# sandialabs/PyNucleus

Hardware: AMD Instinct MI355X
Metric: element-pairs/sec assembled (2D P1 fractional s=0.5, dense) + % fp64 roofline (higher is better)
Workload: dtype f64; 1 GPU; 2D unit disc (uniform_disc refined 7x, 98304 cells), P1, 48769 DoFs, fractional s=0.5, horizon=inf, dense getDense incl. zeroExterior; 4831887360 element pairs/step; noRef=7, num_dofs=48769, num_cells=98304, parallelism=block rows of the upper triangle dealt over 1 GPU(s), row-owned one-sided slabs

## Files before the change

### include/pnl_hip.h

```cpp
#ifndef PNL_HIP_H
#define PNL_HIP_H
#include <stdint.h>

#ifdef __cplusplus
extern "C" {
#endif

typedef struct pnl_context pnl_context;

enum pnl_status {
    PNL_OK = 0,
    PNL_ERR_INVALID = -1,
    PNL_ERR_UNSUPPORTED = -2,
    PNL_ERR_HIP = -3,
    PNL_ERR_STATE = -4,
    PNL_ERR_ORDER = -5
};

enum pnl_kernel_type { PNL_FRACTIONAL = 0, PNL_INDICATOR = 1, PNL_PERIDYNAMIC = 2, PNL_GAUSSIAN = 3, PNL_EXPONENTIAL = 4,
                       PNL_GAUSSIAN_BOUNDARY = 5, PNL_EXPONENTIAL_BOUNDARY = 6 };

typedef struct {
    int32_t ktype;
    int32_t interaction;
// ... 117 lines not shown
int pnl_h2_get(pnl_context *ctx, int which, double *dst_host);
int pnl_h2_set(pnl_context *ctx, int which, const double *src_host);
int pnl_h2_matvec_block(pnl_context *ctx, int nvec, const double *X_dev, int64_t ldx, double *Y_dev, int64_t ldy);
int pnl_h2_upward_block(pnl_context *ctx, int nvec, const double *X_dev, int64_t ldx, double *cupB_dev);
int pnl_h2_interact_block(pnl_context *ctx, const double *cupB_dev, double *cdownB_dev);
int pnl_h2_downward_block(pnl_context *ctx, int nvec, double *cdownB_dev, double *Y_dev, int64_t ldy);

int pnl_spmv(pnl_context *ctx, const double *data_dev, const double *diag_dev, const double *x_dev, double *y_dev);

typedef struct pnl_order_function {
    int32_t type, normalized;
    double p[6];
    int32_t scal_n, pad;
    double scal_mid, scal_half;
    double scal_cheb[32];
} pnl_order_function;

int pnl_set_order_function(pnl_context *ctx, const pnl_order_function *f, const double *cell_smax, const double *facet_smax,
                           double c0, double bc0, double sing_fac, double bsing_fac);
int pnl_set_order_vertex_values(pnl_context *ctx, int nv, const double *values_host);
int pnl_upload_pointwise_rules(pnl_context *ctx, int which, int panel, int nkeys, int M, int rows, const double *nodes,
                               const double *w, const double *phi0, const double *phi1);
int pnl_assemble_dense_pointwise(pnl_context *ctx, double *A, int64_t ldA, int zero_exterior, int cell_begin, int cell_end,
                                 int npairs, const int32_t *pairs, int nbpairs, const int32_t *bpairs);
int pnl_assemble_pairs_masked_pointwise(pnl_context *ctx, int np, const int32_t *pairs, const uint64_t *masks, const int32_t *rule,
                                        double *data);
int pnl_assemble_boundary_masked_pointwise(pnl_context *ctx, int ni, const int32_t *cells, const int32_t *facets, const uint32_t *masks,
                                           const int32_t *rule, const double *sv, double fac, double *data, double *diag);

int pnl_get_counters(pnl_context *ctx, int64_t *out, int n);
int pnl_get_phase_ms(pnl_context *ctx, float *out, int n);
int pnl_get_settled_tiles(pnl_context *ctx, int32_t *tiles, int64_t ntiles);
int pnl_get_settled_lists(pnl_context *ctx, uint16_t *codes, uint16_t *lists, int64_t ntiles);
int pnl_uniform_lane_layout(int nc, const int32_t *cells, const int32_t *dofs, int mode, int nthreads, int32_t *sizes, uint8_t *lane_cell,
                            int16_t *lds_col, int8_t *vorder, int16_t *cell_col, double *mult, double *seconds);
enum pnl_kernel_slot { PNL_K_TILE_GENERAL = 0, PNL_K_TILE_UNIFORM2, PNL_K_TILE_UNIFORM3, PNL_K_TILE_UNIFORM4, PNL_K_FOLD_MIRROR,
                       PNL_K_WORKLIST, PNL_K_TILE_SETTLED, PNL_NUM_KERNEL_SLOTS };
int pnl_get_kernel_ms(pnl_context *ctx, float *out, int n);

typedef struct pnl_tree pnl_tree;
typedef struct pnl_nfplan pnl_nfplan;
int pnl_tree_build(int N, int dim, const double *boxes, const int64_t *d2c_ptr, const int32_t *d2c_idx, int nc, double eta,
                   int min_size, int max_levels, int do_admissibility, pnl_tree **out);
int pnl_tree_build_blocks(int N, int dim, const double *boxes, const int64_t *d2c_ptr, const int32_t *d2c_idx, int nc, double eta,
                          int min_size, int max_levels, int do_admissibility, const int32_t *dof_block, int mixed_block,
                          pnl_tree **out);
int pnl_tree_build_refined(int N, int dim, const double *boxes, const int64_t *d2c_ptr, const int32_t *d2c_idx, int nc, double eta,
                           int min_size, int max_levels, int do_admissibility, const int32_t *dof_block, int mixed_block, int ref_type,
                           pnl_tree **out);
int pnl_tree_build_horizon(int N, int dim, const double *boxes, const int64_t *d2c_ptr, const int32_t *d2c_idx, int nc, double eta,
                           int min_size, int max_levels, int do_admissibility, const int32_t *dof_block, int mixed_block, int ref_type,
                           double horizon, pnl_tree **out);
int pnl_tree_build_device(int N, int dim, const double *boxes, const int64_t *d2c_ptr, const int32_t *d2c_idx, int nc, double eta,
                          int min_size, int max_levels, int do_admissibility, int ref_type, pnl_tree **out);
void pnl_tree_destroy(pnl_tree *T);
int pnl_tree_sizes(const pnl_tree *T, int64_t *out3);
int pnl_tree_get(const pnl_tree *T, int32_t *range, int32_t *parent, int32_t *children, int32_t *level, double *box, int32_t *perm,
                 int32_t *near, int32_t *far);
int pnl_tree_node_cells(const pnl_tree *T, int n, const int32_t *node_ids, int64_t *off, int32_t *cells);
int pnl_h2_transfer_matrices(int nnodes, int dim, int m, const double *box, const int32_t *parent, double *out);
int pnl_nfplan_build(int dim, int nv, const double *vertices, int nc, const int32_t *cells, int dpe, int N, const int32_t *dofs,
                     int nnodes, const int64_t *node_off, const int32_t *node_dofs, const int64_t *node_cell_off,
                     const int32_t *node_cells, int npairs, const int32_t *pair_nodes, int tile, int max_chunk_dofs,
                     pnl_nfplan **out);
void pnl_nfplan_destroy(pnl_nfplan *P);
int pnl_nfplan_sizes(const pnl_nfplan *P, int64_t *out9);
// ... 123 lines not shown
```

### pynucleus_amd/_lib.py

```python
import ctypes as C
import os
import numpy as np

_HERE = os.path.dirname(os.path.abspath(__file__))
LIB_PATH = os.environ.get('PNL_LIB', os.path.join(_HERE, 'libpnl_hip.so'))

PNL_OK = 0
PNL_ERR_INVALID = -1
PNL_ERR_UNSUPPORTED = -2
PNL_ERR_HIP = -3
PNL_ERR_STATE = -4
PNL_ERR_ORDER = -5
PNL_INTERIOR = 0
PNL_BOUNDARY = 1
PNL_FLAG_NO_MIRROR = 1
PNL_FLAG_SYMMETRIC_FLUSH = 2
PNL_NUM_COUNTERS = 140

EXPORTS = ['pnl_create', 'pnl_destroy', 'pnl_error_string', 'pnl_version', 'pnl_set_stream', 'pnl_synchronize',
           'pnl_upload_mesh', 'pnl_upload_dofmap', 'pnl_set_kernel', 'pnl_set_order_formula', 'pnl_upload_distant_rules',
           'pnl_upload_singular_rule', 'pnl_upload_boundary', 'pnl_assemble_dense', 'pnl_dense_overwrites', 'pnl_block_row_costs', 'pnl_tile_cells',
           'pnl_assemble_dense_tiles', 'pnl_get_counters', 'pnl_get_phase_ms', 'pnl_get_kernel_ms', 'pnl_get_settled_tiles', 'pnl_tree_build', 'pnl_tree_build_blocks', 'pnl_tree_build_refined', 'pnl_tree_build_horizon', 'pnl_tree_build_device', 'pnl_tree_destroy', 'pnl_tree_sizes', 'pnl_tree_get', 'pnl_tree_node_cells', 'pnl_h2_transfer_matrices', 'pnl_nfplan_build', 'pnl_nfplan_destroy', 'pnl_nfplan_sizes', 'pnl_nfplan_get', 'pnl_horizon_pattern', 'pnl_near_pattern', 'pnl_pattern_set_max_nnz', 'pnl_set_option', 'pnl_set_cell_order', 'pnl_set_interaction_transform', 'pnl_set_order_vertex_values', 'pnl_h2_get', 'pnl_h2_set', 'pnl_pattern_nnz', 'pnl_pattern_get', 'pnl_pattern_destroy', 'pnl_set_row_slab', 'pnl_diag_blocks_size', 'pnl_get_diag_blocks', 'pnl_slab_matvec', 'pnl_slab_diagonal', 'pnl_gemv', 'pnl_cg_jacobi',
           'pnl_inv_diagonal', 'pnl_set_classes', 'pnl_select_class', 'pnl_upload_sparsity', 'pnl_upload_sparsity_device', 'pnl_assemble_pairs_masked', 'pnl_assemble_boundary_masked', 'pnl_assemble_clusters_tiled', 'pnl_h2_setup', 'pnl_h2_matvec', 'pnl_h2_upward', 'pnl_h2_interact', 'pnl_h2_downward', 'pnl_h2_sizes', 'pnl_spmv',
           'pnl_assemble_pairs_in_horizon', 'pnl_assemble_pairs_in_horizon_range', 'pnl_set_nonsymmetric', 'pnl_set_order_function', 'pnl_upload_pointwise_rules', 'pnl_assemble_dense_pointwise',
           'pnl_assemble_pairs_masked_pointwise', 'pnl_assemble_boundary_masked_pointwise', 'pnl_get_settled_lists',
           'pnl_gemv_axpby', 'pnl_csr_matvec', 'pnl_mg_create', 'pnl_mg_destroy', 'pnl_mg_cycle', 'pnl_mg_solve', 'pnl_mg_cg', 'pnl_theta_step', 'pnl_selftest',
           'pnl_potrf', 'pnl_potrs', 'pnl_getrf', 'pnl_getrs',
           'pnl_csr_cg_jacobi', 'pnl_fe_space_create', 'pnl_fe_space_destroy', 'pnl_assemble_nonlinearity', 'pnl_imex_create',
           'pnl_imex_destroy', 'pnl_imex_sweep', 'pnl_lincomb', 'pnl_gemv_multi', 'pnl_gemv_block', 'pnl_spmv_block', 'pnl_uniform_lane_layout',
           'pnl_h2_matvec_block', 'pnl_h2_upward_block', 'pnl_h2_interact_block', 'pnl_h2_downward_block',
           'pnl_cg_jacobi_block', 'pnl_cgb_init', 'pnl_cgb_update', 'pnl_cgb_refresh', 'pnl_cgb_direction']

PNL_FUN_BRUSSELATOR, PNL_FUN_CUBIC = 0, 1
PNL_IMEX_CG_MG, PNL_IMEX_CHOL = 0, 1
PNL_IMEX_MAX_STAGES, PNL_IMEX_MAX_COMP = 4, 2
PNL_INTERP_MAX_OPS = 21
PNL_CGB_MAXVEC, PNL_CGB_STATE = 16, 8


def source_sha16():
    import glob
    import hashlib
    root = os.path.dirname(_HERE)
    files = sorted(glob.glob(os.path.join(_HERE, 'csrc', '*.h'))+glob.glob(os.path.join(_HERE, 'csrc', '*.hip'))
                   +[os.path.join(root, 'include', 'pnl_hip.h'), os.path.join(_HERE, 'csrc', 'Makefile')])
    h = hashlib.sha256()
    for fn in files:
        with open(fn, 'rb') as f:
            h.update(os.path.basename(fn).encode()+b'\0'+f.read())
    return h.hexdigest()[:16]


class pnl_kernel(C.Structure):
    _fields_ = [('ktype', C.c_int32), ('interaction', C.c_int32), ('exponent', C.c_double), ('scale', C.c_double),
                ('horizon2', C.c_double)]


class pnl_order_formula(C.Structure):
# ... 54 lines not shown
        return _LIB
    if not os.path.exists(LIB_PATH):
        raise PnlError('{} is missing: the HIP extension has not been built (run __graft_entry__.build()); '
                       'there is no CPU fallback for the assembly path'.format(LIB_PATH))
    import torch
    L = C.CDLL(LIB_PATH)
    vp, i32, i64, dbl = C.c_void_p, C.c_int, C.c_int64, C.c_double
    L.pnl_create.argtypes = [i32, C.POINTER(vp)]
    L.pnl_destroy.argtypes = [vp]
    L.pnl_destroy.restype = None
    L.pnl_error_string.argtypes = [vp]
    L.pnl_error_string.restype = C.c_char_p
    L.pnl_version.restype = C.c_char_p
    L.pnl_set_stream.argtypes = [vp, vp]
    L.pnl_synchronize.argtypes = [vp]
    L.pnl_upload_mesh.argtypes = [vp, i32, i32, vp, i32, vp, vp, vp, dbl]
    L.pnl_upload_dofmap.argtypes = [vp, i32, i32, i32, i32, vp, vp]
    L.pnl_set_kernel.argtypes = [vp, i32, C.POINTER(pnl_kernel)]
    L.pnl_selftest.argtypes = [i32, i32, i32, i32, vp, i32, vp, vp]
    L.pnl_set_order_formula.argtypes = [vp, i32, C.POINTER(pnl_order_formula)]
    L.pnl_upload_distant_rules.argtypes = [vp, i32, vp, vp, vp, vp, vp, vp, vp]
    L.pnl_upload_singular_rule.argtypes = [vp, i32, i32, i32, i32, vp, vp, vp, dbl]
    L.pnl_upload_boundary.argtypes = [vp, i32, vp]
    L.pnl_assemble_dense.argtypes = [vp, vp, i64, i32, i32, i32, i32]
    L.pnl_dense_overwrites.argtypes = [vp, i32, i32, i32]
    L.pnl_block_row_costs.argtypes = [vp, vp, i32]
    L.pnl_tile_cells.argtypes = [vp]
    L.pnl_assemble_dense_tiles.argtypes = [vp, vp, i64, i32, i32, vp, i32, i32, i32]
    L.pnl_get_counters.argtypes = [vp, vp, i32]
    L.pnl_get_phase_ms.argtypes = [vp, vp, i32]
    L.pnl_get_kernel_ms.argtypes = [vp, vp, i32]
    L.pnl_get_settled_tiles.argtypes = [vp, vp, C.c_int64]
    L.pnl_get_settled_lists.argtypes = [vp, vp, vp, C.c_int64]
    L.pnl_uniform_lane_layout.argtypes = [i32, vp, vp, i32, i32, vp, vp, vp, vp, vp, vp, vp]
    L.pnl_set_row_slab.argtypes = [vp, i32, vp, i32, vp]
    L.pnl_tree_build.argtypes = [i32, i32, vp, vp, vp, i32, dbl, i32, i32, i32, C.POINTER(vp)]
    L.pnl_tree_build_blocks.argtypes = [i32, i32, vp, vp, vp, i32, dbl, i32, i32, i32, vp, i32, C.POINTER(vp)]
    L.pnl_tree_build_refined.argtypes = [i32, i32, vp, vp, vp, i32, dbl, i32, i32, i32, vp, i32, i32, C.POINTER(vp)]
    L.pnl_tree_build_horizon.argtypes = [i32, i32, vp, vp, vp, i32, dbl, i32, i32, i32, vp, i32, i32, dbl, C.POINTER(vp)]
    L.pnl_tree_build_device.argtypes = [i32, i32, vp, vp, vp, i32, dbl, i32, i32, i32, i32, C.POINTER(vp)]
    L.pnl_tree_destroy.argtypes = [vp]
    L.pnl_tree_destroy.restype = None
    L.pnl_tree_sizes.argtypes = [vp, vp]
    L.pnl_tree_get.argtypes = [vp, vp, vp, vp, vp, vp, vp, vp, vp]
    L.pnl_tree_node_cells.argtypes = [vp, i32, vp, vp, vp]
    L.pnl_h2_transfer_matrices.argtypes = [i32, i32, i32, vp, vp, vp]
    L.pnl_nfplan_build.argtypes = [i32, i32, vp, i32, vp, i32, i32, vp, i32, vp, vp, vp, vp, i32, vp, i32, i32, C.POINTER(vp)]
    L.pnl_nfplan_destroy.argtypes = [vp]
    L.pnl_nfplan_destroy.restype = None
    L.pnl_nfplan_sizes.argtypes = [vp, vp]
    L.pnl_nfplan_get.argtypes = [vp, i32, vp]
    L.pnl_horizon_pattern.argtypes = [i32, i32, vp, i32, vp, i32, i32, vp, dbl, i32, C.POINTER(vp)]
    L.pnl_near_pattern.argtypes = [vp, i32, vp, i32, C.POINTER(vp)]
    L.pnl_pattern_nnz.argtypes = [vp]
    L.pnl_pattern_set_max_nnz.argtypes = [i64]
    L.pnl_set_option.argtypes = [C.c_char_p, C.c_char_p]
    L.pnl_set_cell_order.argtypes = [vp, i32, vp]
    L.pnl_set_interaction_transform.argtypes = [vp, i32, vp]
    L.pnl_set_order_vertex_values.argtypes = [vp, i32, vp]
    L.pnl_h2_get.argtypes = [vp, i32, vp]
    L.pnl_h2_set.argtypes = [vp, i32, vp]
    L.pnl_pattern_get.argtypes = [vp, vp, vp]
    L.pnl_pattern_destroy.argtypes = [vp]
    L.pnl_diag_blocks_size.argtypes = [vp]
    L.pnl_get_diag_blocks.argtypes = [vp, vp]
    L.pnl_slab_matvec.argtypes = [vp, vp, i64, vp, vp, vp]
# ... 409 lines not shown
        self.check(self.L.pnl_get_diag_blocks(self.h, C.c_void_p(dst_ptr)))

    def slab_matvec(self, slab_ptr, ld, dblocks_ptr, x_ptr, y_ptr):
        self.check(self.L.pnl_slab_matvec(self.h, C.c_void_p(slab_ptr), int(ld), C.c_void_p(dblocks_ptr), C.c_void_p(x_ptr), C.c_void_p(y_ptr)))

    def slab_diagonal(self, slab_ptr, ld, dblocks_ptr, diag_ptr):
        self.check(self.L.pnl_slab_diagonal(self.h, C.c_void_p(slab_ptr), int(ld), C.c_void_p(dblocks_ptr), C.c_void_p(diag_ptr)))

    def kernel_ms(self):
        out = np.zeros(7, dtype=np.float32)
        self.check(self.L.pnl_get_kernel_ms(self.h, out.ctypes.data, 7))
        return dict(tile_general=float(out[0]), tile_uniform2=float(out[1]), tile_uniform3=float(out[2]), tile_uniform4=float(out[3]),
                    fold_mirror=float(out[4]), worklist=float(out[5]), tile_settled=float(out[6]))

    def settled_tiles(self):
        n = self.L.pnl_get_settled_tiles(self.h, None, 0)
        self.check(min(n, 0))
        tiles = np.zeros((n, 2), dtype=np.int32)
        if n:
            self.check(min(self.L.pnl_get_settled_tiles(self.h, tiles.ctypes.data, n), 0))
        return tiles

    def settled_lists(self):
        n = self.settled_tiles().shape[0]
        codes = np.zeros((n, 512), dtype=np.uint16)
        have = self.L.pnl_get_settled_lists(self.h, codes.ctypes.data if n else None, None, n)
        self.check(min(have, 0))
        if not have:
            return codes, None
        lists = np.zeros((n, 4104), dtype=np.uint16)
        self.check(min(self.L.pnl_get_settled_lists(self.h, None, lists.ctypes.data, n), 0))
        return codes, lists

    def gemv(self, A_ptr, ldA, n, x_ptr, y_ptr, symmetric_half=False):
        self.check(self.L.pnl_gemv(self.h, C.c_void_p(A_ptr), int(ldA), int(n), C.c_void_p(x_ptr), C.c_void_p(y_ptr),
                                   int(symmetric_half)))

    def cg_jacobi(self, A_ptr, ldA, n, b_ptr, x_ptr, tol, maxiter):
        it, res = C.c_int(0), C.c_double(0.)
        self.check(self.L.pnl_cg_jacobi(self.h, C.c_void_p(A_ptr), int(ldA), int(n), C.c_void_p(b_ptr), C.c_void_p(x_ptr),
                                        float(tol), int(maxiter), C.byref(it), C.byref(res)))
        return it.value, res.value

    def gemv_axpby(self, A_ptr, ldA, nrows, ncols, x_ptr, alpha, beta, b_ptr, y_ptr):
        self.check(self.L.pnl_gemv_axpby(self.h, C.c_void_p(A_ptr), int(ldA), int(nrows), int(ncols), C.c_void_p(x_ptr), float(alpha),
                                         float(beta), C.c_void_p(b_ptr) if b_ptr else None, C.c_void_p(y_ptr)))

    @staticmethod
    def _block_list(A_ptrs, coeffs):
        c = np.ascontiguousarray(coeffs, dtype=np.float64)
        assert c.ndim == 1 and c.shape[0] == len(A_ptrs)
        return (C.c_void_p*max(len(A_ptrs), 1))(*[int(p) if p else None for p in A_ptrs]), c

    def lincomb(self, A_ptrs, ldA, nrows, ncols, coeffs, B_ptr, ldB):
        arr, c = self._block_list(A_ptrs, coeffs)
        self.check(self.L.pnl_lincomb(self.h, len(A_ptrs), arr, int(ldA), int(nrows), int(ncols), c.ctypes.data, C.c_void_p(B_ptr) if B_ptr else None,
                                      int(ldB)))

    def gemv_multi(self, A_ptrs, ldA, nrows, ncols, coeffs, x_ptr, alpha, beta, b_ptr, y_ptr):
        arr, c = self._block_list(A_ptrs, coeffs)
        self.check(self.L.pnl_gemv_multi(self.h, len(A_ptrs), arr, int(ldA), int(nrows), int(ncols), c.ctypes.data, C.c_void_p(x_ptr), float(alpha),
                                         float(beta), C.c_void_p(b_ptr) if b_ptr else None, C.c_void_p(y_ptr)))

    def gemv_block(self, A_ptr, ldA, nrows, ncols, nvec, X_ptr, ldx, alpha, beta, B_ptr, ldb, Y_ptr, ldy):
        self.check(self.L.pnl_gemv_block(self.h, C.c_void_p(A_ptr) if A_ptr else None, int(ldA), int(nrows), int(ncols), int(nvec),
                                         C.c_void_p(X_ptr) if X_ptr else None, int(ldx), float(alpha), float(beta),
# ... 139 lines not shown
```

### pynucleus_amd/csrc/pnl_context.h

```cpp
#pragma once
#include <hip/hip_runtime.h>
#include <algorithm>
#include <cmath>
#include <cstdarg>
#include <cstdio>
#include <cstring>
#include <string>
#include <vector>
#include "pnl_hip.h"
#include "pnl_device.h"

constexpr int TILE_P1 = 64;
constexpr int TILE_P2 = 32;

struct DevBuf {
    void *p = nullptr;
    size_t bytes = 0;
    ~DevBuf() { release(); }
    void release() { if (p) { (void)hipFree(p); p = nullptr; bytes = 0; } }
};

enum PhaseEvent {
    EV_START = 0,
    EV_WORKLIST_DONE = 1,
// ... 45 lines not shown
    double H0 = 0.;
    std::vector<double> vertices, vol, h;
    std::vector<int32_t> cells, dofs, perm_table, bcells;
    struct ClassData {
        pnl_kernel kern[2];
        pnl_order_formula form[2];
        bool have_kernel[2] = {false, false}, have_form[2] = {false, false};
        bool have_sing[2][3] = {{false, false, false}, {false, false, false}};
        DevBuf b_sn[3], b_sw[3], b_sp[3], b_bn[2], b_bw[2], b_bp[2], b_spairs[3], b_bpairs[2], b_spairs1[3];
        int sM[3] = {0, 0, 0}, sRows[3] = {0, 0, 0}, bM[2] = {0, 0};
        double sFac = 0., bFac = 0.;
        int n_spairs[3] = {0, 0, 0}, n_bpairs[2] = {0, 0};
        int n_spairs1[3] = {0, 0, 0};
        ClassData() { std::memset(kern, 0, sizeof(kern)); std::memset(form, 0, sizeof(form)); }
    };
    std::vector<ClassData*> cls;
    int cur = 0;
    ClassData &C() { return *cls[cur]; }
    int nlab = 0;
    bool nonsym = false;
    int orient = 0;
    std::vector<int32_t> cell_labels, facet_labels, cls_of;
    bool have_mesh = false, have_dofs = false, have_rules = false, have_boundary = false;
    bool dirty = true;
    DevProblem P;
    DevBuf b_cellv, b_ccen, b_cvol, b_ch, b_clog, b_cvid, b_cdof, b_cslot, b_blk_ndof, b_blk_dofs, b_perm, b_off, b_bary, b_w, b_phi,
        b_foff, b_fbary, b_fw, b_bvid, b_bv, b_bgeo, b_counters, b_D, b_tiles,
        b_vec[6], b_clabel, b_blabel, b_clsof, b_scal, b_wl, b_wlcount, b_tilectr, b_ttn, b_ttoff, b_tttab, b_ttwphi, b_wlsorted, b_wlaux,
        b_vertices, b_sp_indptr, b_sp_indices, b_mp_pairs, b_mp_masks, b_mp_wl, b_mp_sorted, b_mp_aux, b_bi_cells, b_bi_facets,
        b_bi_masks, b_cp[28], b_cpD, b_wlds, b_wlpair, b_h2[27];
    DevBuf b_kcls, b_fcls, b_uni, b_tilecls, b_ttwphif;
    DevBuf b_scolbase, b_srowoff, b_cpoff, b_cpslot, b_cprow, b_foldtab, b_bkcls, b_bfcls, b_bdefer, b_multitiles, b_slotA, b_candtiles, b_candq;
    int slot_S = 0, n_multitiles = 0;
    DevBuf b_codes, b_lists;
    int n_settled = 0, settled_want = -1, lists_want = -1;
    std::vector<int2> settled_tiles;
    long long code_builds = 0;
    DevBuf b_unictr;
    static constexpr int UNI_CTRS = 64;
    long long slot_total = 0;
    DevBuf b_rowmap, b_rowdof, b_colmap, b_coldof;
    DevBuf b_cholinfo;
    DevBuf b_luwork, b_lutmp;
    DevBuf b_blk_part, b_blk_xt;
    DevBuf b_cgb_part, b_cgb_work;
    std::vector<int32_t> slab_rowdofs, slab_coldofs;
    int slab_rows = 0, slab_cols = 0;
    std::vector<DevKernel> kcls_host;
    std::vector<DevKernel> bkcls_host;
    std::vector<DevFormula> bfcls_host;
    std::vector<DevFormula> fcls_host;
    int uni_off[5] = {-1, -1, -1, -1, -1}, uni_np[5] = {0, 0, 0, 0, 0};
    bool uni_struct[5] = {false, false, false, false, false};
    H2Dev h2;
    bool have_h2 = false;
    bool have_tile_order = false;
    struct TileOrderJob *tile_job = nullptr;
    DevBuf b_cellv_t, b_cdof_t, b_cslot_t, b_Dt;
    UniLaneTables uni_lanes[3];
    int uni_lanes_up = -1;
    double uni_lanes_seconds = 0.;
    DevBuf b_ul_cell, b_ul_col, b_ul_ccol, b_ul_cellv, b_ul_cvol, b_ul_cslot, b_ul_real;
    std::vector<double> ul_cellv_t;
    std::vector<short> ul_cslot_t;
    PwDev pw;
    bool have_pw = false, have_pw_rules[2][3] = {{false, false, false}, {false, false, false}};
// ... 236 lines not shown
```

### pynucleus_amd/csrc/pnl_device.h

```cpp
#pragma once
#include <hip/hip_runtime.h>
#include <stdint.h>

#define PNL_NTHREADS 256
#define PNL_MAXQ 120
#define PNL_NCOUNTERS 136
#define PNL_DC_UNI_TILES_UNCHECKED 134
#define PNL_DC_UNI_TILES_CHECKED 135
#define PNL_WL_SLOTS 256
#define PNL_WL_BINS 128
#define PNL_POW_TAB_DOUBLES 384
#define PNL_TT_MAXPTS 96
#define PNL_GEN_MAXPTS 16

struct DevKernel {
    int ktype;
    int fast;
    double exponent, scale, horizon2;
    int interaction, qm;
    double pb[6];
    const double *ptab;
};

struct DevFormula {
// ... 32 lines not shown
    const double *tt_wphi;
    const double *tt_wphif;
    int tt_npts, pad1;
    int sM[3], sRows[3];
    const double *sNodes[3], *sW[3], *sPsi[3];
    double sFac;
    int bM[2];
    const double *bNodes[2], *bW[2], *bPhi[2];
    double bFac;
    const int *bvid;
    const double *bv;
    const double *bgeo;
    const int *clabel, *blabel, *cls_of;
    int nlab, cur_class;
    int orient, pad2;
    double idfac;
    unsigned long long *counters;
    const int *rowmap, *colmap;
    int onesided, pad3;
    const double *uni = nullptr;
    int uni_off[5] = {0, 0, 0, 0, 0};
    int mix_struct = 0;
};

constexpr int PNL_DIAG_MULT = 21;
#define PNL_LIST_HEAD 8
#define PNL_LIST_STRIDE (PNL_LIST_HEAD+4096)
__host__ __device__ constexpr int tile_sweep_row(int tid, int k, int tile, int nt) { return k*(nt/tile)+tid/tile; }
__host__ __device__ constexpr int tile_diag_cell(int r, int j, int tile) { return (r+PNL_DIAG_MULT*j)%tile; }

__device__ __forceinline__ long long pnl_row(const DevProblem &P, int I) { return P.rowmap ? (long long)P.rowmap[I] : (long long)I; }
__device__ __forceinline__ int pnl_col(const DevProblem &P, int J) { return P.colmap ? P.colmap[J] : J; }

#define PNL_FOLD_TAB 63
struct FoldEntry { long long off; int ar, cy; };

struct H2Dev {
    int dim, m, M, nnodes, nleaves, nfar;
    const double *box;
    const int *parent;
    const int *leaf_node;
    const int *leaf_dof_off, *leaf_dofs;
    const int *leaf_cell_off, *leaf_cells;
    const long long *leaf_val_off;
    const int *far;
    double *V, *K;
    const double *T;
    double *cup, *cdown;
};

__device__ __forceinline__ double cheb_node(double a, double b, int m, int j) {
    return (b-a)*0.5*(cos((2.0*(m-j)-1.0)/(2.0*m)*3.14159265358979323846)+1.0)+a;
}

__device__ __forceinline__ double lagrange1d(double a, double b, int m, int l, double x) {
    const double xl = cheb_node(a, b, m, l);
    double v = 1.;
    for (int k = 0; k < m; k++)
        if (k != l) {
            const double xk = cheb_node(a, b, m, k);
            v *= (x-xk)/(xl-xk);
        }
    return v;
}

struct PwDev {
    int type, normalized;
// ... 38 lines not shown
```

### pynucleus_amd/csrc/pnl_setup.hip

```cpp
#include <hip/hip_runtime.h>
#include <algorithm>
#include <chrono>
#include <cmath>
#include <cstdio>
#include <cstring>
#include <deque>
#include <map>
#include <mutex>
#include <string>
#include <thread>
#include <vector>
#include "pnl_hip.h"
#include "pnl_context.h"

template <class F>
static void host_threads(F body, int want = 0) {
    const int nthr = want > 0 ? std::min(want, 64) : (int)std::max(1u, std::min(8u, std::thread::hardware_concurrency()));
    std::vector<std::thread> pool;
    for (int th = 0; th < nthr; th++) pool.emplace_back([&body, th, nthr]() { body(th, nthr); });
    for (auto &t : pool) t.join();
}

struct TileOrderJob {
    std::vector<int> cells, lperm;
// ... 576 lines not shown
}

static int upload_slot_tables(pnl_context *ctx, const CellTables &F) {
    int rc;
    const int nblocks = F.nblocks;
    const std::vector<std::vector<int>> &lists = F.lists;
    const std::vector<int32_t> &blk_ndof = F.blk_ndof;
    std::vector<int32_t> colbase(nblocks+1, 0);
    for (int b = 0; b < nblocks; b++) colbase[b+1] = colbase[b]+((blk_ndof[b]+7) & ~7);
    const int S = colbase[nblocks];
    std::vector<long long> rowoff(nblocks, 0);
    long long run = 0;
    for (int a = 0; a < nblocks; a++) { rowoff[a] = run; run += (long long)blk_ndof[a]*(S-colbase[a]); }
    ctx->slot_S = S; ctx->slot_total = run;
    std::vector<int32_t> cpoff(ctx->N+1, 0);
    for (int b = 0; b < nblocks; b++) for (int g : lists[b]) cpoff[g+1]++;
    for (int g = 0; g < ctx->N; g++) cpoff[g+1] += cpoff[g];
    std::vector<int2> cp(cpoff[ctx->N]);
    std::vector<int32_t> fillp(cpoff.begin(), cpoff.end()-1);
    std::vector<long long> cprow(cp.size());
    for (int b = 0; b < nblocks; b++)
        for (size_t r = 0; r < lists[b].size(); r++) {
            const int k = fillp[lists[b][r]]++;
            cp[k] = make_int2(b, colbase[b]+(int)r);
            cprow[k] = rowoff[b]+(long long)r*(S-colbase[b])-colbase[b];
        }
    if ((rc = upload(ctx, ctx->b_cprow, cprow.data(), cprow.size()))) return rc;
    if ((rc = upload(ctx, ctx->b_scolbase, colbase.data(), colbase.size()))) return rc;
    if ((rc = upload(ctx, ctx->b_srowoff, rowoff.data(), rowoff.size()))) return rc;
    if ((rc = upload(ctx, ctx->b_cpoff, cpoff.data(), cpoff.size()))) return rc;
    if ((rc = upload(ctx, ctx->b_cpslot, cp.data(), cp.size()))) return rc;
    const int nranges = (ctx->N+31)/32;
    std::vector<FoldEntry> tab((size_t)nranges*(PNL_FOLD_TAB+1));
    for (int q = 0; q < nranges; q++) {
        FoldEntry *e = &tab[(size_t)q*(PNL_FOLD_TAB+1)];
        const int g0 = cpoff[q*32], g1 = cpoff[std::min(ctx->N, q*32+32)];
        e[0].off = g1-g0; e[0].ar = 0; e[0].cy = 0;
        if (g1-g0 > PNL_FOLD_TAB) continue;
        for (int I = q*32; I < std::min(ctx->N, q*32+32); I++)
            for (int g = cpoff[I]; g < cpoff[I+1]; g++) {
                FoldEntry &x = e[1+g-g0];
                x.off = cprow[g]; x.ar = (cp[g].x << 5) | (I-q*32); x.cy = cp[g].y;
            }
    }
    return upload(ctx, ctx->b_foldtab, tab.data(), tab.size());
}

static void fill_problem(pnl_context *ctx, const CellTables &F) {
    const int dim = F.dim, dpe = F.dpe, nc = F.nc, ncp = F.ncp, nblocks = F.nblocks, nU = ctx->nU, nlab = ctx->nlab;
    DevProblem &P = ctx->P;
    P.dim = dim; P.dpe = dpe; P.nc = nc; P.ncp = ncp; P.N = ctx->N; P.dpv = ctx->dpv; P.dped = ctx->dped; P.nb = ctx->nb;
    P.H0 = ctx->H0;
    P.cellv = (const double*)ctx->b_cellv.p; P.ccen = (const double*)ctx->b_ccen.p;
    P.cvol = (const double*)ctx->b_cvol.p; P.ch = (const double*)ctx->b_ch.p; P.clog = (const double*)ctx->b_clog.p;
    P.cvid = (const int*)ctx->b_cvid.p; P.cdof = (const int*)ctx->b_cdof.p; P.cslot = (const short*)ctx->b_cslot.p;
    P.blk_ndof = (const int*)ctx->b_blk_ndof.p; P.blk_dofs = (const int*)ctx->b_blk_dofs.p;
    P.blk_stride = nU; P.nblocks = nblocks;
    P.perm_table = (const int*)ctx->b_perm.p;
    P.bvid = (const int*)ctx->b_bvid.p; P.bv = (const double*)ctx->b_bv.p; P.bgeo = (const double*)ctx->b_bgeo.p;
    P.counters = (unsigned long long*)ctx->b_counters.p;
    P.nlab = nlab; P.cur_class = -1; P.orient = 0; P.pad2 = 0; P.idfac = 1.;
    P.clabel = (const int*)ctx->b_clabel.p; P.blabel = (const int*)ctx->b_blabel.p; P.cls_of = (const int*)ctx->b_clsof.p;
}

static int finalize(pnl_context *ctx) {
    if (!ctx->dirty) return PNL_OK;
    if (!ctx->have_mesh || !ctx->have_dofs) return fail(ctx, PNL_ERR_STATE, "mesh and DoF map must be uploaded first");
    const int dim = ctx->dim, nV = dim+1, nc = ctx->nc, dpe = ctx->dpe;
    if (!((dim == 2 && (dpe == 1 || dpe == 3 || dpe == 6)) || (dim == 1 && dpe >= 1 && dpe <= 4)))
        return fail(ctx, PNL_ERR_UNSUPPORTED, "unsupported (dim=%d, dofs_per_element=%d)", dim, dpe);
    const int T = ctx->tile = (dpe == 6 || (dim == 1 && dpe >= 3)) ? TILE_P2 : TILE_P1;
    const int nblocks = ctx->nblocks = (nc+T-1)/T;
    const int ncp = ctx->ncp = nblocks*T;
    CellTables F;
    F.dim = dim; F.nV = nV; F.nc = nc; F.dpe = dpe; F.T = T; F.nblocks = nblocks; F.ncp = ncp;
    tile_order_drop(ctx);
    int rc;
// ... 962 lines not shown

int pnl_get_phase_ms(pnl_context *ctx, float *out, int n) {
    if (!ctx || !out || n <= 0) return PNL_ERR_INVALID;
    if (!ctx->run.ev_valid) return fail(ctx, PNL_ERR_STATE, "nothing assembled yet");
    HIPCHK(ctx, hipEventSynchronize(ctx->ev[EV_END]));
    float t[7] = {0, 0, 0, 0, 0, 0, 0}, tmp;
    if (ctx->run.tiles_launched) {
        HIPCHK(ctx, hipEventElapsedTime(&t[0], ctx->ev[EV_START], ctx->ev[EV_TILES_DONE]));
        HIPCHK(ctx, hipEventElapsedTime(&t[1], ctx->ev[EV_TILES_DONE], ctx->ev[EV_WORKLIST_DONE]));
        if (ctx->run.pure_launched && ctx->cls.size() == 1) {
            HIPCHK(ctx, hipEventElapsedTime(&t[6], ctx->ev[EV_START], ctx->ev[EV_TILES_UNIFORM_DONE]));
            t[0] -= t[6];
        }
    }
    HIPCHK(ctx, hipEventElapsedTime(&tmp, ctx->ev[EV_WORKLIST_DONE], ctx->ev[EV_MIRROR_DONE]));
    HIPCHK(ctx, hipEventElapsedTime(&t[2], ctx->ev[EV_MIRROR_DONE], ctx->ev[EV_SINGULAR_DONE]));
    HIPCHK(ctx, hipEventElapsedTime(&t[3], ctx->ev[EV_SINGULAR_DONE], ctx->ev[EV_BOUNDARY_DONE]));
    HIPCHK(ctx, hipEventElapsedTime(&t[4], ctx->ev[EV_BOUNDARY_DONE], ctx->ev[EV_END]));
    t[4] += tmp;
    HIPCHK(ctx, hipEventElapsedTime(&t[5], ctx->ev[EV_START], ctx->ev[EV_END]));
    for (int i = 0; i < n && i < 7; i++) out[i] = t[i];
    return PNL_OK;
}

int pnl_get_settled_tiles(pnl_context *ctx, int32_t *tiles, int64_t ntiles) {
    if (!ctx || ntiles < 0 || (ntiles && !tiles)) return PNL_ERR_INVALID;
    if (!ctx->b_tiles.p || ctx->cls_n_mixed.empty()) return fail(ctx, PNL_ERR_STATE, "no tile plan yet");
    const std::vector<int2> &st = ctx->settled_tiles;
    if ((int)st.size() != ctx->n_settled) return fail(ctx, PNL_ERR_STATE, "the resident tile list is not that of a dense assembly");
    for (size_t i = 0; i < st.size() && (int64_t)i < ntiles; i++) { tiles[2*i] = st[i].x; tiles[2*i+1] = st[i].y; }
    return (int)st.size();
}

int pnl_get_settled_lists(pnl_context *ctx, uint16_t *codes, uint16_t *lists, int64_t ntiles) {
    if (!ctx || ntiles < 0) return PNL_ERR_INVALID;
    if (!ctx->b_tiles.p || ctx->cls_n_mixed.empty()) return fail(ctx, PNL_ERR_STATE, "no tile plan yet");
    const int64_t n = std::min<int64_t>(ntiles, ctx->n_settled);
    HIPCHK(ctx, hipStreamSynchronize(ctx->stream));
    if (codes && n > 0) HIPCHK(ctx, hipMemcpy(codes, ctx->b_codes.p, (size_t)n*512*sizeof(uint16_t), hipMemcpyDeviceToHost));
    if (lists && n > 0) {
        if (!ctx->b_lists.p) return fail(ctx, PNL_ERR_STATE, "the resident tile plan keeps no pair lists");
        HIPCHK(ctx, hipMemcpy(lists, ctx->b_lists.p, (size_t)n*PNL_LIST_STRIDE*sizeof(uint16_t), hipMemcpyDeviceToHost));
    }
    return ctx->b_lists.p ? ctx->n_settled : 0;
}

int pnl_uniform_lane_layout(int nc, const int32_t *cells, const int32_t *dofs, int mode, int nthreads, int32_t *sizes, uint8_t *lane_cell,
                            int16_t *lds_col, int8_t *vorder, int16_t *cell_col, double *mult, double *seconds) {
    if (nc <= 0 || !cells || !dofs || !sizes || mode < 0 || mode > 2) return PNL_ERR_INVALID;
    const int T = 64, nblocks = (nc+T-1)/T, ncp = nblocks*T;
    std::vector<int16_t> cslot((size_t)3*ncp, -1);
    std::vector<std::vector<int>> lists(nblocks);
    int nU = 1;
    for (int b = 0; b < nblocks; b++) {
        auto &L = lists[b];
        for (int c = b*T; c < std::min(nc, (b+1)*T); c++) for (int k = 0; k < 3; k++) if (dofs[(size_t)c*3+k] >= 0) L.push_back(dofs[(size_t)c*3+k]);
        std::sort(L.begin(), L.end());
        L.erase(std::unique(L.begin(), L.end()), L.end());
        nU = std::max<int>(nU, (int)L.size());
    }
    sizes[0] = nblocks; sizes[1] = nU; sizes[2] = mode == 0 ? 0 : 16*uni_lane_cap(nU)+16; sizes[3] = ncp;
    if (!lane_cell || !lds_col || !vorder || !cell_col || !mult) return PNL_OK;
    std::vector<int> cl(cells, cells+(size_t)nc*3), lperm((size_t)nc*3);
    for (int c = 0; c < nc; c++) for (int k = 0; k < 3; k++) lperm[(size_t)c*3+k] = k;
    host_threads([&](int th, int nthr) {
        for (int b = th; b < nblocks; b += nthr) tile_order_block(b, nc, T, cl.data(), lperm.data());
// ... 37 lines not shown
```

### pynucleus_amd/csrc/pnl_tile2.h

```cpp
#pragma once
#include "pnl_common.h"

__host__ __device__ constexpr int uni_rule_size(int dpe, int np) { return 3*np+np+np*dpe+(dpe*(dpe+1)/2)*np; }


template <bool NT>
__global__ void __launch_bounds__(256)
k_fold_mirror(const double *__restrict__ A2, const FoldEntry *__restrict__ tab, const int *__restrict__ cpoff, const int2 *__restrict__ cp,
              const long long *__restrict__ cprow, double *__restrict__ A, long long ldA, int N) {
    __shared__ double t1[32][33], t2[32][33];
    __shared__ FoldEntry s_tab[2][PNL_FOLD_TAB+1];
    const unsigned nb = (unsigned)(N+31)/32;
    const unsigned nbs = (nb+7)/8;
    const unsigned sbid = blockIdx.x >> 6, inner = blockIdx.x & 63;
    unsigned I;
    {
        const float t = 2.f*(float)nbs+1.f;
        const float fb = (t-sqrtf(fmaxf(t*t-8.f*(float)sbid, 0.f)))*0.5f;
        I = (unsigned)fmaxf(fb, 0.f);
        if (I >= nbs) I = nbs-1;
        while (I > 0 && I*nbs-I*(I-1)/2 > sbid) I--;
        while (I+1 < nbs && (I+1)*nbs-(I+1)*I/2 <= sbid) I++;
    }
    const unsigned J = I+(sbid-(I*nbs-I*(I-1)/2));
    const unsigned bi = 8*I+(inner >> 3), bj = 8*J+(inner & 7);
    if (bi > bj || bj >= nb) return;
    const int tid = threadIdx.x, tx = tid & 31, ty = tid >> 5;
    if (tid < 2*(PNL_FOLD_TAB+1)) {
        const int side = tid >= PNL_FOLD_TAB+1, k = tid-side*(PNL_FOLD_TAB+1);
        s_tab[side][k] = tab[(size_t)(side ? bj : bi)*(PNL_FOLD_TAB+1)+k];
    }
    for (int k = tid; k < 32*33; k += 256) { (&t1[0][0])[k] = 0.; (&t2[0][0])[k] = 0.; }
    __syncthreads();
    const int n0 = (int)s_tab[0][0].off, n1 = (int)s_tab[1][0].off;
    if (n0 <= PNL_FOLD_TAB && n1 <= PNL_FOLD_TAB) {
#pragma unroll
        for (int g = 0; g < 2; g++) {
            if (g && bi == bj) break;
            const int nr = g ? n1 : n0, nc = g ? n0 : n1;
            double *__restrict__ tf = g ? &t2[0][0] : &t1[0][0];
            const unsigned total = (unsigned)(nr*nc), inv = ((1u << 20)+(unsigned)nc-1u)/(unsigned)nc;
            for (unsigned base = 0; base < total; base += 8*256) {
                double v[8];
                int dst[8];
#pragma unroll
                for (int u = 0; u < 8; u++) {
                    const unsigned idx = base+256u*u+(unsigned)tid;
                    dst[u] = -1;
                    v[u] = 0.;
                    if (idx < total) {
                        const unsigned ci = (idx*inv) >> 20, cj = idx-ci*(unsigned)nc;
                        const FoldEntry rw = s_tab[g][1+ci], col = s_tab[1-g][1+cj];
                        if ((col.ar >> 5) >= (rw.ar >> 5)) { v[u] = A2[rw.off+col.cy]; dst[u] = (rw.ar & 31)*33+(col.ar & 31); }
                    }
                }
#pragma unroll
                for (int u = 0; u < 8; u++) if (dst[u] >= 0) lds_add_f64(tf+dst[u], v[u]);
            }
        }
    } else {
        auto gather = [&](int br, int bc, double (*t)[33]) {
            const int J = min(bc*32+tx, N), j0 = cpoff[J], j1 = cpoff[min(J+1, N)];
#pragma unroll 1
            for (int rr = 0; rr < 4; rr++) {
                const int r = ty+8*rr, I = min(br*32+r, N);
                double s = 0.;
                for (int ci = cpoff[I]; ci < cpoff[min(I+1, N)]; ci++) {
                    const int a = cp[ci].x;
                    const double *__restrict__ rowp = A2+cprow[ci];
                    for (int cj = j0; cj < j1; cj++) {
                        const int2 c2 = cp[cj];
                        if (c2.x >= a) s += rowp[c2.y];
                    }
                }
                t[r][tx] = s;
            }
        };
        gather((int)bi, (int)bj, t1);
        if (bi != bj) gather((int)bj, (int)bi, t2);
    }
    __syncthreads();
    for (int r = ty; r < 32; r += 8) {
        const int I = bi*32+r, J = bj*32+tx;
        if (I < N && J < N) {
            const double v = (bi != bj) ? t1[r][tx]+t2[tx][r] : ((r != tx) ? t1[r][tx]+t1[tx][r] : t1[r][tx]);
            if (NT) __builtin_nontemporal_store(v, A+(long long)I*ldA+J); else A[(long long)I*ldA+J] = v;
        }
        const int I2 = bj*32+r, J2 = bi*32+tx;
        if (bi != bj && I2 < N && J2 < N) {
            const double v = t2[r][tx]+t1[tx][r];
// ... 1071 lines not shown
```

Before: 67.05 billion element-pairs/s.

## Restructure fold-mirror kernel with wave-broadcast row entries and sorted fold tables

Rewrites the fast path of the fold-mirror kernel. Instead of staging fold tables in shared memory and decoding flat indices by division, each wave now holds row entries in lanes and broadcasts them with readlane, while each lane owns a column entry. The fold table capacity is doubled so more 32-DoF ranges take the packed path instead of the slow gather fallback. Entries are sorted by column and carry block-range bounds, so whole g-passes with no overlap are skipped. It also adds debug and export APIs for the slot tables and a standalone fold call, and risks more register pressure and a larger table footprint.

```diff
diff --git a/include/pnl_hip.h b/include/pnl_hip.h
--- a/include/pnl_hip.h
+++ b/include/pnl_hip.h
@@ -173,6 +173,8 @@
 int pnl_get_phase_ms(pnl_context *ctx, float *out, int n);
 int pnl_get_settled_tiles(pnl_context *ctx, int32_t *tiles, int64_t ntiles);
 int pnl_get_settled_lists(pnl_context *ctx, uint16_t *codes, uint16_t *lists, int64_t ntiles);
+int pnl_get_slot_tables(pnl_context *ctx, int64_t *sizes, int32_t *blk_ndof, int32_t *blk_dofs, int32_t *colbase, int64_t *rowoff);
+int pnl_fold_slots(pnl_context *ctx, const double *slots_dev, double *A_dev, int64_t ldA);
 int pnl_uniform_lane_layout(int nc, const int32_t *cells, const int32_t *dofs, int mode, int nthreads, int32_t *sizes, uint8_t *lane_cell,
                             int16_t *lds_col, int8_t *vorder, int16_t *cell_col, double *mult, double *seconds);
 enum pnl_kernel_slot { PNL_K_TILE_GENERAL = 0, PNL_K_TILE_UNIFORM2, PNL_K_TILE_UNIFORM3, PNL_K_TILE_UNIFORM4, PNL_K_FOLD_MIRROR,
diff --git a/pynucleus_amd/_lib.py b/pynucleus_amd/_lib.py
--- a/pynucleus_amd/_lib.py
+++ b/pynucleus_amd/_lib.py
@@ -24,6 +24,7 @@
            'pnl_inv_diagonal', 'pnl_set_classes', 'pnl_select_class', 'pnl_upload_sparsity', 'pnl_upload_sparsity_device', 'pnl_assemble_pairs_masked', 'pnl_assemble_boundary_masked', 'pnl_assemble_clusters_tiled', 'pnl_h2_setup', 'pnl_h2_matvec', 'pnl_h2_upward', 'pnl_h2_interact', 'pnl_h2_downward', 'pnl_h2_sizes', 'pnl_spmv',
            'pnl_assemble_pairs_in_horizon', 'pnl_assemble_pairs_in_horizon_range', 'pnl_set_nonsymmetric', 'pnl_set_order_function', 'pnl_upload_pointwise_rules', 'pnl_assemble_dense_pointwise',
            'pnl_assemble_pairs_masked_pointwise', 'pnl_assemble_boundary_masked_pointwise', 'pnl_get_settled_lists',
+           'pnl_get_slot_tables', 'pnl_fold_slots',
            'pnl_gemv_axpby', 'pnl_csr_matvec', 'pnl_mg_create', 'pnl_mg_destroy', 'pnl_mg_cycle', 'pnl_mg_solve', 'pnl_mg_cg', 'pnl_theta_step', 'pnl_selftest',
            'pnl_potrf', 'pnl_potrs', 'pnl_getrf', 'pnl_getrs',
            'pnl_csr_cg_jacobi', 'pnl_fe_space_create', 'pnl_fe_space_destroy', 'pnl_assemble_nonlinearity', 'pnl_imex_create',
@@ -144,6 +145,8 @@
     L.pnl_get_kernel_ms.argtypes = [vp, vp, i32]
     L.pnl_get_settled_tiles.argtypes = [vp, vp, C.c_int64]
     L.pnl_get_settled_lists.argtypes = [vp, vp, vp, C.c_int64]
+    L.pnl_get_slot_tables.argtypes = [vp, vp, vp, vp, vp, vp]
+    L.pnl_fold_slots.argtypes = [vp, vp, vp, i64]
     L.pnl_uniform_lane_layout.argtypes = [i32, vp, vp, i32, i32, vp, vp, vp, vp, vp, vp, vp]
     L.pnl_set_row_slab.argtypes = [vp, i32, vp, i32, vp]
     L.pnl_tree_build.argtypes = [i32, i32, vp, vp, vp, i32, dbl, i32, i32, i32, C.POINTER(vp)]
@@ -619,6 +622,22 @@
         self.check(min(self.L.pnl_get_settled_lists(self.h, None, lists.ctypes.data, n), 0))
         return codes, lists
 
+    def slot_tables(self):
+        sizes = np.zeros(8, dtype=np.int64)
+        self.check(self.L.pnl_get_slot_tables(self.h, sizes.ctypes.data, None, None, None, None))
+        nblocks, nU = int(sizes[0]), int(sizes[1])
+        blk_ndof = np.zeros(nblocks, dtype=np.int32)
+        blk_dofs = np.zeros((nblocks, nU), dtype=np.int32)
+        colbase = np.zeros(nblocks+1, dtype=np.int32)
+        rowoff = np.zeros(nblocks, dtype=np.int64)
+        self.check(self.L.pnl_get_slot_tables(self.h, sizes.ctypes.data, blk_ndof.ctypes.data, blk_dofs.ctypes.data, colbase.ctypes.data,
+                                              rowoff.ctypes.data))
+        return dict(nblocks=nblocks, nU=nU, S=int(sizes[2]), total=int(sizes[3]), capacity=int(sizes[4]), most=int(sizes[5]),
+                    over=int(sizes[6]), N=int(sizes[7]), blk_ndof=blk_ndof, blk_dofs=blk_dofs, colbase=colbase, rowoff=rowoff)
+
+    def fold_slots(self, slots_ptr, A_ptr, ldA):
+        self.check(self.L.pnl_fold_slots(self.h, C.c_void_p(slots_ptr), C.c_void_p(A_ptr), int(ldA)))
+
     def gemv(self, A_ptr, ldA, n, x_ptr, y_ptr, symmetric_half=False):
         self.check(self.L.pnl_gemv(self.h, C.c_void_p(A_ptr), int(ldA), int(n), C.c_void_p(x_ptr), C.c_void_p(y_ptr),
                                    int(symmetric_half)))
diff --git a/pynucleus_amd/csrc/pnl_context.h b/pynucleus_amd/csrc/pnl_context.h
--- a/pynucleus_amd/csrc/pnl_context.h
+++ b/pynucleus_amd/csrc/pnl_context.h
@@ -101,6 +101,7 @@
     DevBuf b_kcls, b_fcls, b_uni, b_tilecls, b_ttwphif;
     DevBuf b_scolbase, b_srowoff, b_cpoff, b_cpslot, b_cprow, b_foldtab, b_bkcls, b_bfcls, b_bdefer, b_multitiles, b_slotA, b_candtiles, b_candq;
     int slot_S = 0, n_multitiles = 0;
+    int fold_most = 0, fold_over = 0;
     DevBuf b_codes, b_lists;
     int n_settled = 0, settled_want = -1, lists_want = -1;
     std::vector<int2> settled_tiles;
diff --git a/pynucleus_amd/csrc/pnl_device.h b/pynucleus_amd/csrc/pnl_device.h
--- a/pynucleus_amd/csrc/pnl_device.h
+++ b/pynucleus_amd/csrc/pnl_device.h
@@ -88,7 +88,7 @@
 __device__ __forceinline__ long long pnl_row(const DevProblem &P, int I) { return P.rowmap ? (long long)P.rowmap[I] : (long long)I; }
 __device__ __forceinline__ int pnl_col(const DevProblem &P, int J) { return P.colmap ? P.colmap[J] : J; }
 
-#define PNL_FOLD_TAB 63
+#define PNL_FOLD_TAB 127
 struct FoldEntry { long long off; int ar, cy; };
 
 struct H2Dev {
diff --git a/pynucleus_amd/csrc/pnl_setup.hip b/pynucleus_amd/csrc/pnl_setup.hip
--- a/pynucleus_amd/csrc/pnl_setup.hip
+++ b/pynucleus_amd/csrc/pnl_setup.hip
@@ -632,17 +632,26 @@
     if ((rc = upload(ctx, ctx->b_cpslot, cp.data(), cp.size()))) return rc;
     const int nranges = (ctx->N+31)/32;
     std::vector<FoldEntry> tab((size_t)nranges*(PNL_FOLD_TAB+1));
+    int most = 0, over = 0;
     for (int q = 0; q < nranges; q++) {
         FoldEntry *e = &tab[(size_t)q*(PNL_FOLD_TAB+1)];
         const int g0 = cpoff[q*32], g1 = cpoff[std::min(ctx->N, q*32+32)];
         e[0].off = g1-g0; e[0].ar = 0; e[0].cy = 0;
-        if (g1-g0 > PNL_FOLD_TAB) continue;
+        most = std::max(most, g1-g0);
+        if (g1-g0 > PNL_FOLD_TAB) { over++; continue; }
+        int n = 0;
         for (int I = q*32; I < std::min(ctx->N, q*32+32); I++)
             for (int g = cpoff[I]; g < cpoff[I+1]; g++) {
-                FoldEntry &x = e[1+g-g0];
-                x.off = cprow[g]; x.ar = (cp[g].x << 5) | (I-q*32); x.cy = cp[g].y;
-            }
-    }
+                FoldEntry &x = e[1+n++];
+                x.off = cprow[g]*(long long)sizeof(double); x.ar = (cp[g].x << 5) | (I-q*32); x.cy = cp[g].y;
+            }
+        std::sort(e+1, e+1+n, [](const FoldEntry &x, const FoldEntry &y) { return x.cy < y.cy; });
+        if (n) { e[0].ar = e[1].ar >> 5; e[0].cy = e[n].ar >> 5; }
+    }
+    ctx->fold_most = most; ctx->fold_over = over;
+    if (pnl_tune("PNL_VERBOSE"))
+        fprintf(stderr, "[pnl] fold tables: %d ranges of 32 DoFs, at most %d copies in one, %d above the packed capacity of %d\n", nranges, most, over,
+                PNL_FOLD_TAB);
     return upload(ctx, ctx->b_foldtab, tab.data(), tab.size());
 }
 
@@ -1671,6 +1680,32 @@
     return (int)st.size();
 }
 
+int pnl_get_slot_tables(pnl_context *ctx, int64_t *sizes, int32_t *blk_ndof, int32_t *blk_dofs, int32_t *colbase, int64_t *rowoff) {
+    if (!ctx || !sizes) return PNL_ERR_INVALID;
+    if (!ctx->have_mesh || !ctx->have_dofs) return fail(ctx, PNL_ERR_STATE, "mesh and DoF map must be uploaded first");
+    if (int rc = finalize(ctx)) return rc;
+    const int nblocks = ctx->nblocks, nU = ctx->nU;
+    sizes[0] = nblocks; sizes[1] = nU; sizes[2] = ctx->slot_S; sizes[3] = ctx->slot_total; sizes[4] = PNL_FOLD_TAB;
+    sizes[5] = ctx->fold_most; sizes[6] = ctx->fold_over; sizes[7] = ctx->N;
+    HIPCHK(ctx, hipStreamSynchronize(ctx->stream));
+    if (blk_ndof) HIPCHK(ctx, hipMemcpy(blk_ndof, ctx->b_blk_ndof.p, sizeof(int32_t)*(size_t)nblocks, hipMemcpyDeviceToHost));
+    if (blk_dofs) HIPCHK(ctx, hipMemcpy(blk_dofs, ctx->b_blk_dofs.p, sizeof(int32_t)*(size_t)nblocks*nU, hipMemcpyDeviceToHost));
+    if (colbase) HIPCHK(ctx, hipMemcpy(colbase, ctx->b_scolbase.p, sizeof(int32_t)*(size_t)(nblocks+1), hipMemcpyDeviceToHost));
+    if (rowoff) HIPCHK(ctx, hipMemcpy(rowoff, ctx->b_srowoff.p, sizeof(int64_t)*(size_t)nblocks, hipMemcpyDeviceToHost));
+    return PNL_OK;
+}
+
+int pnl_fold_slots(pnl_context *ctx, const double *slots_dev, double *A_dev, int64_t ldA) {
+    if (!ctx || !slots_dev || !A_dev) return PNL_ERR_INVALID;
+    if (!ctx->have_mesh || !ctx->have_dofs) return fail(ctx, PNL_ERR_STATE, "mesh and DoF map must be uploaded first");
+    if (int rc = finalize(ctx)) return rc;
+    if (ldA < ctx->N) return fail(ctx, PNL_ERR_INVALID, "ldA = %lld is smaller than the %d DoFs", (long long)ldA, ctx->N);
+    pnl_begin_assembly(ctx);
+    SlotOut SO = slot_out(ctx);
+    SO.A2 = const_cast<double*>(slots_dev);
+    return pnl2_fold_mirror(ctx, SO, A_dev, ldA);
+}
+
 int pnl_get_settled_lists(pnl_context *ctx, uint16_t *codes, uint16_t *lists, int64_t ntiles) {
     if (!ctx || ntiles < 0) return PNL_ERR_INVALID;
     if (!ctx->b_tiles.p || ctx->cls_n_mixed.empty()) return fail(ctx, PNL_ERR_STATE, "no tile plan yet");
diff --git a/pynucleus_amd/csrc/pnl_tile2.h b/pynucleus_amd/csrc/pnl_tile2.h
--- a/pynucleus_amd/csrc/pnl_tile2.h
+++ b/pynucleus_amd/csrc/pnl_tile2.h
@@ -9,7 +9,6 @@
 k_fold_mirror(const double *__restrict__ A2, const FoldEntry *__restrict__ tab, const int *__restrict__ cpoff, const int2 *__restrict__ cp,
               const long long *__restrict__ cprow, double *__restrict__ A, long long ldA, int N) {
     __shared__ double t1[32][33], t2[32][33];
-    __shared__ FoldEntry s_tab[2][PNL_FOLD_TAB+1];
     const unsigned nb = (unsigned)(N+31)/32;
     const unsigned nbs = (nb+7)/8;
     const unsigned sbid = blockIdx.x >> 6, inner = blockIdx.x & 63;
@@ -26,36 +25,48 @@
     const unsigned bi = 8*I+(inner >> 3), bj = 8*J+(inner & 7);
     if (bi > bj || bj >= nb) return;
     const int tid = threadIdx.x, tx = tid & 31, ty = tid >> 5;
-    if (tid < 2*(PNL_FOLD_TAB+1)) {
-        const int side = tid >= PNL_FOLD_TAB+1, k = tid-side*(PNL_FOLD_TAB+1);
-        s_tab[side][k] = tab[(size_t)(side ? bj : bi)*(PNL_FOLD_TAB+1)+k];
-    }
+    const int lane = tid & 63, wv = __builtin_amdgcn_readfirstlane(tid >> 6);
+    const FoldEntry *__restrict__ const tab0 = tab+(size_t)bi*(PNL_FOLD_TAB+1), *__restrict__ const tab1 = tab+(size_t)bj*(PNL_FOLD_TAB+1);
+    const FoldEntry h0 = tab0[0], h1 = tab1[0];
+    const int rsel = 1+min(wv+4*lane, PNL_FOLD_TAB-1);
+    FoldEntry row = tab0[rsel], col = tab1[1+lane];
     for (int k = tid; k < 32*33; k += 256) { (&t1[0][0])[k] = 0.; (&t2[0][0])[k] = 0.; }
     __syncthreads();
-    const int n0 = (int)s_tab[0][0].off, n1 = (int)s_tab[1][0].off;
+    const int n0 = (int)h0.off, n1 = (int)h1.off;
     if (n0 <= PNL_FOLD_TAB && n1 <= PNL_FOLD_TAB) {
 #pragma unroll
         for (int g = 0; g < 2; g++) {
             if (g && bi == bj) break;
+            if ((g ? h0.cy : h1.cy) < (g ? h1.ar : h0.ar)) continue;
+            const FoldEntry *__restrict__ const ct = g ? tab0 : tab1;
+            if (g) { row = tab1[rsel]; col = tab0[1+lane]; }
             const int nr = g ? n1 : n0, nc = g ? n0 : n1;
-            double *__restrict__ tf = g ? &t2[0][0] : &t1[0][0];
-            const unsigned total = (unsigned)(nr*nc), inv = ((1u << 20)+(unsigned)nc-1u)/(unsigned)nc;
-            for (unsigned base = 0; base < total; base += 8*256) {
-                double v[8];
-                int dst[8];
-#pragma unroll
-                for (int u = 0; u < 8; u++) {
-                    const unsigned idx = base+256u*u+(unsigned)tid;
-                    dst[u] = -1;
-                    v[u] = 0.;
-                    if (idx < total) {
-                        const unsigned ci = (idx*inv) >> 20, cj = idx-ci*(unsigned)nc;
-                        const FoldEntry rw = s_tab[g][1+ci], col = s_tab[1-g][1+cj];
-                        if ((col.ar >> 5) >= (rw.ar >> 5)) { v[u] = A2[rw.off+col.cy]; dst[u] = (rw.ar & 31)*33+(col.ar & 31); }
+            double *__restrict__ const tf = g ? &t2[0][0] : &t1[0][0];
+            const int rar = wv+4*lane < nr ? row.ar : 0x7fffffff, rlo = (int)row.off, rhi = (int)(row.off >> 32);
+            const int nrw = (nr-wv+3) >> 2;
+            constexpr int FB = 8;
+            for (int c0 = 0; c0 < nc; c0 += 64) {
+                if (c0) col = ct[1+min(c0+lane, PNL_FOLD_TAB-1)];
+                const int cblk = c0+lane < nc ? col.ar >> 5 : -1;
+                const unsigned cbyte = (unsigned)col.cy*(unsigned)sizeof(double);
+                double *__restrict__ const cdst = tf+(col.ar & 31);
+                for (int k0 = 0; k0 < nrw; k0 += FB) {
+                    double v[FB];
+                    int dst[FB];
+                    bool ok[FB];
+#pragma unroll
+                    for (int u = 0; u < FB; u++) {
+                        const int ar = __builtin_amdgcn_readlane(rar, k0+u);
+                        const int2 o2 = make_int2(__builtin_amdgcn_readlane(rlo, k0+u), __builtin_amdgcn_readlane(rhi, k0+u));
+                        const long long off = __builtin_bit_cast(long long, o2);
+                        ok[u] = cblk >= (ar >> 5);
+                        dst[u] = (ar & 31)*33;
+                        const char *__restrict__ const rowp = (const char*)A2+off;
+                        if (ok[u]) v[u] = *(const double*)(rowp+cbyte);
                     }
-                }
-#pragma unroll
-                for (int u = 0; u < 8; u++) if (dst[u] >= 0) lds_add_f64(tf+dst[u], v[u]);
+#pragma unroll
+                    for (int u = 0; u < FB; u++) if (ok[u]) lds_add_f64(cdst+dst[u], v[u]);
+                }
             }
         }
     } else {
```

After: 67.72 billion element-pairs/s, median of 6. About the same (+1.0%).
